# mp3guy/Kintinuous

Hardware: AMD Instinct MI355X
Metric: RGB-D frames/sec @640x480, 512^3 TSDF (higher is better)
Workload: dtype f32; 1 GPU; orbit512: 640x480 synthetic orbit sequence, ICP-only tracking, 512^3 TSDF, inputs resident in HBM, 1 stream per GPU (BASELINE.json configs[1]), log playback with 1 frame of read-ahead; volume=512, cols=640, rows=480, unique_frames=120, pose_gather_bytes=56384, side_gate=0, odometry_fallbacks=0

## Files before the change

kintinuous_amd/csrc/kt_track.hip:

```cpp
#include "kt_internal.hpp"

#include <string.h>
#include <stdlib.h>
#include <float.h>
#include <math.h>

#define KT_RED_THREADS 1024
#define KT_RED_BLOCKS 256
#define KT_VT_TOTAL 8192
#define KT_KBATCH 40
#define KT_P2_PAIRS 4
#define KT_RED_SLOTS 32

template <int CTRL>
__device__ __forceinline__ float kt_dpp(float v)
{
    return __int_as_float(__builtin_amdgcn_update_dpp(0, __float_as_int(v), CTRL, 0xf, 0xf, true));
}
__device__ __forceinline__ float kt_warp32_sum(float v)
{
    v += __int_as_float(__builtin_amdgcn_ds_swizzle(__float_as_int(v), 0x401F));
    v += kt_dpp<0x108>(v);
    v += kt_dpp<0x104>(v);
    v += kt_dpp<0x102>(v);
    v += kt_dpp<0x101>(v);
    return v;
}

__device__ __constant__ unsigned char KT_PA[28] = {0, 0, 0, 0, 0, 0, 0, 1, 1, 1, 1, 1, 1, 2, 2, 2, 2, 2, 3, 3, 3, 3, 4, 4, 4, 5, 5, 6};
__device__ __constant__ unsigned char KT_PB[28] = {0, 1, 2, 3, 4, 5, 6, 1, 2, 3, 4, 5, 6, 2, 3, 4, 5, 6, 3, 4, 5, 6, 4, 5, 6, 5, 6, 6};

struct kt_no_prefetch { __device__ __forceinline__ void operator()() const {} };
#define KT_RED_PAIRS 15
#define KT_GRANULE_SENTINEL 0xffffffffffffffffull
#define KT_LEVEL_SETS 2
#define KT_LEVEL_SET_STRIDE 4096
#define KT_LEVEL_SET_BASE 32768
#define KT_POSE_ABORT 15
__device__ __forceinline__ int kt_granule_index(int pair, int wg) { return pair * KT_RED_BLOCKS + (wg & 3) * (KT_RED_BLOCKS / 4) + (wg >> 2); }
__device__ __forceinline__ void kt_publish_pair(unsigned long long* __restrict__ granules, float wsum)
{
    unsigned int lo = __float_as_uint(wsum), hi = (unsigned int)__builtin_amdgcn_readlane((int)__float_as_uint(wsum), 32);
    lo = lo == 0xffffffffu ? 0xfffffffeu : lo;
    const int pair = threadIdx.x >> 6;
    if ((threadIdx.x & 63) == 0 && pair < KT_RED_PAIRS)
        __hip_atomic_store(&granules[kt_granule_index(pair, blockIdx.x)], ((unsigned long long)hi << 32) | (unsigned long long)lo, __ATOMIC_RELAXED,
                           __HIP_MEMORY_SCOPE_AGENT);
}
typedef float kt_rows_t[8][32][2];
static_assert(KT_KBATCH % (2 * KT_P2_PAIRS) == 0, "phase 2 reads whole groups of k-pairs: the staging array must hold them");

typedef float kt_f2 __attribute__((ext_vector_type(2)));
__device__ __forceinline__ float2 kt_lds_pair(const float (&p)[2])
{
    const kt_f2 w = *(const volatile __attribute__((address_space(3))) kt_f2*)p;
    return make_float2(w.x, w.y);
}
template <int NS>
__device__ __forceinline__ void kt_phase2(float (&acc)[NS], const kt_rows_t* const (&rows)[NS], int my_a, int my_b, int vt, int kcount, int kend)
{
    for (int j0 = 0; 2 * j0 < kcount; j0 += KT_P2_PAIRS) {
        float2 ra[KT_P2_PAIRS][NS], rb[KT_P2_PAIRS][NS];
#pragma unroll
        for (int u = 0; u < KT_P2_PAIRS; ++u)
#pragma unroll
            for (int s = 0; s < NS; ++s) {
                ra[u][s] = kt_lds_pair(rows[s][j0 + u][my_a][vt]);
                rb[u][s] = kt_lds_pair(rows[s][j0 + u][my_b][vt]);
            }
#pragma unroll
        for (int u = 0; u < KT_P2_PAIRS; ++u) {
            const int kl = 2 * (j0 + u);
#pragma unroll
            for (int s = 0; s < NS; ++s) acc[s] = kl < kend ? __builtin_fmaf(ra[u][s].x, rb[u][s].x, acc[s]) : acc[s];
#pragma unroll
            for (int s = 0; s < NS; ++s) acc[s] = kl + 1 < kend ? __builtin_fmaf(ra[u][s].y, rb[u][s].y, acc[s]) : acc[s];
        }
    }
}

template <typename RowFn>
__device__ __forceinline__ void kt_reduce29_publish(const RowFn& fn, int n, unsigned long long* __restrict__ granules, kt_rows_t* rows)
{
    KT_TS(0);
    const int tid = threadIdx.x;
    const int t0 = blockIdx.x * 32;
    const int comp = tid >> 5, vt = tid & 31;
    const int my_a = comp < 28 ? KT_PA[comp] : 7, my_b = comp < 28 ? KT_PB[comp] : 7;
    const int nk_vt = (n - (t0 + vt) + KT_VT_TOTAL - 1) / KT_VT_TOTAL;
    const int nk_blk = (n - t0 + KT_VT_TOTAL - 1) / KT_VT_TOTAL;
    float acc[1] = {0.f};
    const kt_rows_t* const rs[1] = {rows};
    for (int kb = 0; kb < nk_blk; kb += KT_KBATCH) {
        const int kcount = min(KT_KBATCH, nk_blk - kb);
        for (int p = tid; p < kcount * 32; p += 2 * KT_RED_THREADS) {
            const int p2 = p + KT_RED_THREADS;
            const int kl = p >> 5, v = p & 31, kl2 = p2 >> 5;
            const int i = t0 + v + (kb + kl) * KT_VT_TOTAL;
            const int i2 = t0 + v + (kb + kl2) * KT_VT_TOTAL;
            const bool has2 = p2 < kcount * 32;
            float row[7], row2[7];
            const bool found = fn(min(i, n - 1), row) && i < n;
            if (__builtin_amdgcn_ballot_w64(has2) != 0) {
                const bool found2 = fn(min(i2, n - 1), row2) && i2 < n && has2;
                if (has2) {
#pragma unroll
                    for (int q = 0; q < 7; ++q) rows[kl2 >> 1][q][v][kl2 & 1] = found2 ? row2[q] : 0.0f;
                    rows[kl2 >> 1][7][v][kl2 & 1] = found2 ? 1.0f : 0.0f;
                }
            }
#pragma unroll
            for (int q = 0; q < 7; ++q) rows[kl >> 1][q][v][kl & 1] = found ? row[q] : 0.0f;
            rows[kl >> 1][7][v][kl & 1] = found ? 1.0f : 0.0f;
        }
        __syncthreads();
        KT_TS_PHASE2(0);
        if (comp < 29) kt_phase2<1>(acc, rs, my_a, my_b, vt, kcount, min(kcount, nk_vt - kb));
        __syncthreads();
        KT_TS_PHASE2(1);
    }
    KT_TS(1);
    const float wsum = kt_warp32_sum(acc[0]);
    kt_publish_pair(granules, wsum);
    KT_TS(2);
}

template <typename RowFnA, typename RowFnB>
__device__ __forceinline__ void kt_reduce29_publish2(const RowFnA& fa, const RowFnB& fb, int n, unsigned long long* __restrict__ granules_a,
                                                     unsigned long long* __restrict__ granules_b, kt_rows_t* rows_a, kt_rows_t* rows_b)
{
    KT_TS(0);
    const int tid = threadIdx.x;
    const int t0 = blockIdx.x * 32;
    const int comp = tid >> 5, vt = tid & 31;
    const int my_a = comp < 28 ? KT_PA[comp] : 7, my_b = comp < 28 ? KT_PB[comp] : 7;
    const int nk_vt = (n - (t0 + vt) + KT_VT_TOTAL - 1) / KT_VT_TOTAL;
    const int nk_blk = (n - t0 + KT_VT_TOTAL - 1) / KT_VT_TOTAL;
    float acc[2] = {0.f, 0.f};
    const kt_rows_t* const rs[2] = {rows_a, rows_b};
    for (int kb = 0; kb < nk_blk; kb += KT_KBATCH) {
        const int kcount = min(KT_KBATCH, nk_blk - kb);
        for (int p = tid; p < kcount * 32; p += KT_RED_THREADS) {
            const int kl = p >> 5, v = p & 31;
            const int i = t0 + v + (kb + kl) * KT_VT_TOTAL;
            const int ii = min(i, n - 1);
            const auto term = fb.fetch_term(ii);
            f3 vcurr, ncurr, vcurr_g, vprev_g, nprev_g;
            bool inimg;
            int g;
            fa.fetch_curr(ii, vcurr, ncurr);
            typename RowFnB::taps tp;
            fb.fetch_taps(term, tp);
            fa.project(vcurr, vcurr_g, inimg, g);
            fa.fetch_prev(g, vprev_g, nprev_g);
            {
                float rb[7];
                const bool found_b = fb.finish(term, tp, rb) && i < n;
#pragma unroll
                for (int q = 0; q < 7; ++q) rows_b[kl >> 1][q][v][kl & 1] = found_b ? rb[q] : 0.0f;
                rows_b[kl >> 1][7][v][kl & 1] = found_b ? 1.0f : 0.0f;
            }
            float ra[7];
            const bool found_a = fa.finish(ncurr, vcurr_g, vprev_g, nprev_g, inimg, ra) && i < n;
#pragma unroll
            for (int q = 0; q < 7; ++q) rows_a[kl >> 1][q][v][kl & 1] = found_a ? ra[q] : 0.0f;
            rows_a[kl >> 1][7][v][kl & 1] = found_a ? 1.0f : 0.0f;
        }
        __syncthreads();
        KT_TS_PHASE2(0);
        if (comp < 29) kt_phase2<2>(acc, rs, my_a, my_b, vt, kcount, min(kcount, nk_vt - kb));
        __syncthreads();
        KT_TS_PHASE2(1);
    }
    KT_TS(1);
    const float wsum_a = kt_warp32_sum(acc[0]), wsum_b = kt_warp32_sum(acc[1]);
    kt_publish_pair(granules_a, wsum_a);
    kt_publish_pair(granules_b, wsum_b);
    KT_TS(2);
}

__device__ unsigned int kt_sweep_spin_limit = 1u << 22;
__device__ unsigned int kt_wait_limit_ticks = 5000000u;
__device__ __forceinline__ unsigned long long kt_ticks() { return __builtin_amdgcn_s_memrealtime(); }

template <int NS>
__device__ __forceinline__ void kt_reduce29_sweep_n(unsigned long long* const (&granules)[NS], float* const (&total)[NS], unsigned int patience = 40u)
{
    const int tid = threadIdx.x;
    KT_TS(3);
    __shared__ unsigned int timed_out;
    if (tid == 0) timed_out = 0;
    __syncthreads();
    {
        const int w = (tid >> 6) - 1, lane = tid & 63;
        if (w >= 0 && w < KT_RED_PAIRS) {
            unsigned long long g[NS][4];
            bool ok;
            unsigned int spins = 0;
            const unsigned int spin_limit = *(volatile const unsigned int*)&kt_sweep_spin_limit;
            const unsigned long long tick_limit = (unsigned long long)*(volatile const unsigned int*)&kt_wait_limit_ticks * patience;
            unsigned long long tick0 = 0;
            for (;;) {
#pragma unroll
                for (int s = 0; s < NS; ++s) {
                    const unsigned long long* pp = &granules[s][w * KT_RED_BLOCKS + lane];
#pragma unroll
                    for (int q = 0; q < 4; ++q) g[s][q] = __hip_atomic_load(pp + q * (KT_RED_BLOCKS / 4), __ATOMIC_RELAXED, __HIP_MEMORY_SCOPE_AGENT);
                }
                ok = true;
#pragma unroll
                for (int s = 0; s < NS; ++s)
#pragma unroll
                    for (int q = 0; q < 4; ++q) ok = ok && g[s][q] != KT_GRANULE_SENTINEL;
                if (__all(ok) || ++spins > spin_limit) break;
                if ((spins & 15u) == 0) {
                    const unsigned long long now = kt_ticks();
                    if (spins == 16u) tick0 = now;
                    else if (now - tick0 > tick_limit) break;
                }
                __builtin_amdgcn_s_sleep(1);
            }
            const bool all_ok = __all(ok);
            if (all_ok) {
#pragma unroll
                for (int s = 0; s < NS; ++s)
#pragma unroll
                    for (int q = 0; q < 4; ++q)
                        __hip_atomic_store(&granules[s][w * KT_RED_BLOCKS + lane + q * (KT_RED_BLOCKS / 4)], KT_GRANULE_SENTINEL, __ATOMIC_RELAXED, __HIP_MEMORY_SCOPE_AGENT);
            }
#pragma unroll
            for (int s = 0; s < NS; ++s)
#pragma unroll
                for (int r = 0; r < 2; ++r) {
                    const int c = 2 * w + r;
                    const float s0 = __uint_as_float((unsigned int)(g[s][0] >> (32 * r))) + 0.0f;
                    const float s1 = __uint_as_float((unsigned int)(g[s][1] >> (32 * r))) + 0.0f;
                    const float s2 = __uint_as_float((unsigned int)(g[s][2] >> (32 * r))) + 0.0f;
                    const float s3 = __uint_as_float((unsigned int)(g[s][3] >> (32 * r))) + 0.0f;
                    const float blk = (s0 + s2) + (s1 + s3);
                    const float tr = kt_warp32_sum(0.0f + blk);
                    const float lo = __int_as_float(__builtin_amdgcn_readlane(__float_as_int(tr), 0));
                    const float hi = __int_as_float(__builtin_amdgcn_readlane(__float_as_int(tr), 32));
                    if (lane == 0 && c < 29) total[s][c] = (lo + 0.0f) + (hi + 0.0f);
                }
            if (lane == 0 && !all_ok) atomicOr(&timed_out, 1u);
        }
    }
    __syncthreads();
    if (tid == 0) total[NS - 1][KT_RED_SLOTS - 1] = timed_out ? 1.0f : 0.0f;
    __syncthreads();
    KT_TS(4);
}

__device__ __forceinline__ void kt_reduce29_sweep(unsigned long long* __restrict__ granules, float (&total)[KT_RED_SLOTS], unsigned int patience = 40u)
{
    unsigned long long* const gs[1] = {granules};
    float* const ts[1] = {total};
    kt_reduce29_sweep_n<1>(gs, ts, patience);
}

#define KT_RED_GRID KT_RED_BLOCKS
__device__ __forceinline__ bool kt_red_publishes() { return true; }
__device__ __forceinline__ bool kt_red_sweeps() { return blockIdx.x == KT_RED_GRID - 1; }

template <typename RowFn, typename PreFn = kt_no_prefetch>
__device__ __forceinline__ bool kt_reduce29(const RowFn& fn, int n, unsigned long long* __restrict__ granules, float (&total)[KT_RED_SLOTS],
                                            const PreFn& pre = PreFn())
{
    __shared__ kt_rows_t rows[KT_KBATCH / 2];
    if (kt_red_publishes()) kt_reduce29_publish(fn, n, granules, rows);
    if (!kt_red_sweeps()) return false;
    pre();
    kt_reduce29_sweep(granules, total);
    return true;
}

int kt_refill_granules(kt_ctx* c)
{
    KT_HIP(hipMemsetAsync(c->red_partials, 0xff, sizeof(double) * 32 * c->red_max_blocks, c->stream));
    return KT_OK;
}

static unsigned int kt_next_epoch(kt_ctx* c)
{
    if (++c->red_epoch >= 0xffffffffu) {
        (void)kt_refill_granules(c);
        c->red_epoch = 1;
    }
    return c->red_epoch;
}
static unsigned long long* kt_residual_granules(kt_ctx* c) { return (unsigned long long*)c->red_partials + 64 * KT_RED_BLOCKS; }
static unsigned int* kt_residual_partials(kt_ctx* c) { return (unsigned int*)((unsigned long long*)c->red_partials + 64 * KT_RED_BLOCKS + 1024); }
static unsigned long long* kt_second_granules(kt_ctx* c) { return (unsigned long long*)c->red_partials + 32 * KT_RED_BLOCKS; }

struct kt_icp_args {
    const float* vmap_curr; const float* nmap_curr;
    const float* vmap_g_prev; const float* nmap_g_prev;
    kt_intr intr;
    int cols, rows;
    float dist_thres, angle_thres;
    float dist2_le, sine2_le;
    kt_mat33 Rcurr; float tcurr[3];
    kt_mat33 Rprev_inv; float tprev[3];
    kt_track_state* state;
    int first;
    unsigned long long* granules; unsigned int fault;
    float* out29;
    int mode;
    int keep29;
    int n_iter; unsigned int seq0; unsigned long long* pose_gran; unsigned long long* level_gran;
    int n_levels;
    struct level { const float* vmap_curr; const float* nmap_curr; const float* vmap_g_prev; const float* nmap_g_prev; kt_intr intr; int cols, rows, n_iter; } lv[KT_LEVELS];
};

struct kt_icp_row {
    struct view { const float* vmap_curr; const float* nmap_curr; const float* vmap_g_prev; const float* nmap_g_prev; kt_intr intr; int cols, rows; float dist2_le, sine2_le; } a;
    kt_mat33 Rcurr, Rprev_inv;
    f3 tcurr, tprev;
    __device__ __forceinline__ explicit kt_icp_row(const kt_icp_args& k)
        : a{k.vmap_curr, k.nmap_curr, k.vmap_g_prev, k.nmap_g_prev, k.intr, k.cols, k.rows, k.dist2_le, k.sine2_le} {}
    __device__ __forceinline__ void set_level(const kt_icp_args::level& v)
    {
        a.vmap_curr = v.vmap_curr; a.nmap_curr = v.nmap_curr; a.vmap_g_prev = v.vmap_g_prev; a.nmap_g_prev = v.nmap_g_prev;
        a.intr = v.intr; a.cols = v.cols; a.rows = v.rows;
    }
    int pf_i = -1;
    f3 pf_v = {0.f, 0.f, 0.f}, pf_n = {0.f, 0.f, 0.f};
    __device__ __forceinline__ void fetch_curr(int i, f3& vcurr, f3& ncurr) const
    {
        const int plane = a.cols * a.rows;
        vcurr = {a.vmap_curr[i], a.vmap_curr[i + plane], a.vmap_curr[i + 2 * plane]};
        ncurr = {a.nmap_curr[i], a.nmap_curr[i + plane], a.nmap_curr[i + 2 * plane]};
    }
    __device__ __forceinline__ void project(const f3& vcurr, f3& vcurr_g, bool& inimg, int& g) const
    {
        const int cols = a.cols, rows = a.rows;
        vcurr_g = kt_add(kt_mul(Rcurr, vcurr), tcurr);
        const f3 vcurr_cp = kt_mul(Rprev_inv, kt_sub(vcurr_g, tprev));
        const int ux = kt_f2i_rn(vcurr_cp.x * a.intr.fx / vcurr_cp.z + a.intr.cx);
        const int uy = kt_f2i_rn(vcurr_cp.y * a.intr.fy / vcurr_cp.z + a.intr.cy);
        inimg = !(ux < 0 || uy < 0 || ux >= cols || uy >= rows || vcurr_cp.z < 0);
        g = inimg ? (int)kt_mad24((unsigned int)uy, (unsigned int)cols, (unsigned int)ux) : 0;
    }
    __device__ __forceinline__ void fetch_prev(int g, f3& vprev_g, f3& nprev_g) const
    {
        const int plane = a.cols * a.rows;
        vprev_g = {a.vmap_g_prev[g], a.vmap_g_prev[g + plane], a.vmap_g_prev[g + 2 * plane]};
        nprev_g = {a.nmap_g_prev[g], a.nmap_g_prev[g + plane], a.nmap_g_prev[g + 2 * plane]};
    }
    __device__ __forceinline__ bool finish(const f3& ncurr, const f3& vcurr_g, const f3& vprev_g, const f3& nprev_g, bool inimg, float (&row)[7]) const
    {
        const f3 ncurr_g = kt_mul(Rcurr, ncurr);
        const f3 dv = kt_sub(vprev_g, vcurr_g);
        const float dist2 = kt_dot(dv, dv);
        const f3 cr = kt_cross(ncurr_g, nprev_g);
        const float sine2 = kt_dot(cr, cr);
        const bool found = inimg && (sine2 <= a.sine2_le && dist2 <= a.dist2_le && !kt_isnan(ncurr.x) && !kt_isnan(nprev_g.x));
        const f3 s_cp = kt_mul(Rprev_inv, kt_sub(vcurr_g, tprev));
        const f3 d_cp = kt_mul(Rprev_inv, kt_sub(vprev_g, tprev));
        const f3 n_cp = kt_mul(Rprev_inv, nprev_g);
        const f3 sxn = kt_cross(s_cp, n_cp);
        row[0] = found ? n_cp.x : 0.0f; row[1] = found ? n_cp.y : 0.0f; row[2] = found ? n_cp.z : 0.0f;
        row[3] = found ? sxn.x : 0.0f; row[4] = found ? sxn.y : 0.0f; row[5] = found ? sxn.z : 0.0f;
        row[6] = found ? kt_dot(n_cp, kt_sub(s_cp, d_cp)) : 0.0f;
        return found;
    }
    __device__ __forceinline__ bool operator()(int i, float (&row)[7]) const
    {
        f3 vcurr, ncurr, vcurr_g, vprev_g, nprev_g;
        bool inimg;
        int g;
        if (i == pf_i) { vcurr = pf_v; ncurr = pf_n; }
        else fetch_curr(i, vcurr, ncurr);
        project(vcurr, vcurr_g, inimg, g);
        fetch_prev(g, vprev_g, nprev_g);
        return finish(ncurr, vcurr_g, vprev_g, nprev_g, inimg, row);
    }
};

extern "C" float kt_debug_sq_threshold(float T, int strict)
{
    if (!(T >= 0.0f) || (strict && !(T > 0.0f))) return -1.0f;
    if (T == INFINITY) return strict ? FLT_MAX : INFINITY;
    const auto ok = [&](float x) { const float r = sqrtf(x); return strict ? r < T : r <= T; };
    float x = T * T;
    if (x == INFINITY) x = FLT_MAX;
    while (x > 0.0f && !ok(x)) x = nextafterf(x, -INFINITY);
    if (!ok(x)) return -1.0f;
    while (x < FLT_MAX && ok(nextafterf(x, INFINITY))) x = nextafterf(x, INFINITY);
    return x;
}
static void kt_icp_set_thresholds(kt_icp_args& a, float dist_thres, float angle_thres)
{
    a.dist_thres = dist_thres; a.angle_thres = angle_thres;
    a.dist2_le = kt_debug_sq_threshold(dist_thres, 0);
    a.sine2_le = kt_debug_sq_threshold(angle_thres, 1);
}

__global__ __launch_bounds__(KT_RED_THREADS) void kt_icp_kernel(const kt_icp_args a)
{
    if (a.fault && blockIdx.x == 0) return;
    kt_icp_row fn(a);
    if (a.state && !a.first) {
        for (int k = 0; k < 9; ++k) { fn.Rcurr.m[k] = a.state->Rcurr[k]; fn.Rprev_inv.m[k] = a.state->Rprev_inv[k]; }
        fn.tcurr = {a.state->tcurr[0], a.state->tcurr[1], a.state->tcurr[2]};
        fn.tprev = {a.state->tprev[0], a.state->tprev[1], a.state->tprev[2]};
    } else {
        fn.Rcurr = a.Rcurr; fn.Rprev_inv = a.Rprev_inv;
        fn.tcurr = {a.tcurr[0], a.tcurr[1], a.tcurr[2]};
        fn.tprev = {a.tprev[0], a.tprev[1], a.tprev[2]};
    }
    __shared__ float total[KT_RED_SLOTS];
    kt_pose_stage ps;
    const bool solve_here = a.mode == KT_MODE_ICP_SOLVE;
    auto pre = [&]() { if (solve_here && !a.first) ps.fetch(a.state); };
    if (!kt_reduce29(fn, a.cols * a.rows, a.granules, total, pre)) return;
    __shared__ double sys[KT_SYS_DOUBLES], pose_d[KT_POSE_STAGE_DOUBLES], tail_work[KT_TAIL_WORK_DOUBLES];
    __shared__ float pose_f[KT_POSE_STAGE_FLOATS];
    if (solve_here) {
        if (threadIdx.x < 42) sys[threadIdx.x] = (double)total[kt_sys_slot(threadIdx.x)];
        if (!a.first) ps.park(pose_d, pose_f);
        else if (threadIdx.x == 64) {
#pragma unroll
            for (int k = 0; k < 16; ++k) pose_d[k] = (k % 5 == 0) ? 1.0 : 0.0;
#pragma unroll
            for (int k = 0; k < 9; ++k) pose_f[k] = a.Rcurr.m[k];
#pragma unroll
            for (int k = 0; k < 3; ++k) pose_f[9 + k] = a.tprev[k];
        }
        __syncthreads();
    }
    if (a.mode == KT_MODE_HOST) {
        if (threadIdx.x < KT_RED_SLOTS && (threadIdx.x < 29 || threadIdx.x == KT_RED_SLOTS - 1)) a.out29[threadIdx.x] = total[threadIdx.x];
    } else if (a.mode == KT_MODE_ICP_SOLVE) {
        if (threadIdx.x == 64) {
            a.state->last_residual[0] = total[27];
            a.state->last_residual[1] = total[28];
            if (a.keep29)
                for (int k = 0; k < 29; ++k) a.state->icp29[k] = total[k];
            if (a.first) {
#pragma unroll
                for (int k = 0; k < 9; ++k) { a.state->Rprev[k] = a.Rcurr.m[k]; a.state->Rprev_inv[k] = a.Rprev_inv.m[k]; }
#pragma unroll
                for (int k = 0; k < 3; ++k) a.state->tprev[k] = a.tprev[k];
                a.state->handoff_timeout = total[KT_RED_SLOTS - 1] != 0.0f ? 1 : 0;
            } else if (total[KT_RED_SLOTS - 1] != 0.0f) {
                a.state->handoff_timeout = 1;
            }
        }
        if (threadIdx.x < 64) {
            kt_solve_and_update_wave(a.state, sys, pose_d, pose_f, tail_work);
#ifdef KT_ICP_TIMING
            if (threadIdx.x == 0) { const unsigned long long t5 = wall_clock64(); for (int q = 0; q < 7; ++q) a.state->icp29[q] = (float)(kt_ts[q + 0] - kt_ts[0]); a.state->icp29[7] = (float)(t5 - kt_ts[0]); }
#endif
        }
    } else if (threadIdx.x == 0) {
        for (int k = 0; k < 29; ++k) a.state->icp29[k] = total[k];
        if (total[KT_RED_SLOTS - 1] != 0.0f) a.state->handoff_timeout = 1;
    }
}


__device__ __forceinline__ void kt_level_wait_pose(const kt_icp_args& a, unsigned int want, float* s_pose)
{
    const int lane = (int)(threadIdx.x & 63u);
    const unsigned int spin_limit = min(*(volatile const unsigned int*)&kt_sweep_spin_limit, 1u << 20);
    const unsigned long long tick_limit = 2ull * *(volatile const unsigned int*)&kt_wait_limit_ticks;
    unsigned long long tick0 = 0;
    unsigned long long g = 0;
    unsigned int spins = 0;
    bool ok, gone;
    for (;;) {
        if (lane < 13) g = __hip_atomic_load(&a.pose_gran[lane == 12 ? KT_POSE_ABORT : lane], __ATOMIC_RELAXED, __HIP_MEMORY_SCOPE_AGENT);
        const int ahead = (int)((unsigned int)(g >> 32) - want);
        ok = lane >= 12 || ahead == 0;
        gone = lane == 12 && ahead >= 0 && ahead < a.n_iter;
        if (__all(ok) || __any(gone) || ++spins > spin_limit) break;
        if ((spins & 15u) == 0) {
            const unsigned long long now = kt_ticks();
            if (spins == 16u) tick0 = now;
// ... 844 lines not shown
```

Baseline: 4257 frames/s.

## Pack two outer-product components per thread in ICP reduction phase 2 with shared slot loads

Phase 2 of the 29-term ICP reduction now assigns each 64-lane wave two pairs of products, drawn from a constexpr table. Each thread loads three component slots and forms two FMAs from them, so LDS reads are shared across products instead of two loads per product. The loop is double-buffered with sched barriers and uses an inline-asm FMA. The per-thread kend bounds check is replaced by zero-padding the staging array in phase 1. Only 8 waves work in phase 2, which concentrates the work and adds table complexity and a padding pass.

New measurement: 4221 frames/s. About the same (-0.9%).

```diff
diff --git a/kintinuous_amd/csrc/kt_track.hip b/kintinuous_amd/csrc/kt_track.hip
--- a/kintinuous_amd/csrc/kt_track.hip
+++ b/kintinuous_amd/csrc/kt_track.hip
@@ -9,7 +9,7 @@
 #define KT_RED_BLOCKS 256
 #define KT_VT_TOTAL 8192
 #define KT_KBATCH 40
-#define KT_P2_PAIRS 4
+#define KT_P2_PAIRS 2
 #define KT_RED_SLOTS 32
 
 template <int CTRL>
@@ -27,8 +27,57 @@
     return v;
 }
 
-__device__ __constant__ unsigned char KT_PA[28] = {0, 0, 0, 0, 0, 0, 0, 1, 1, 1, 1, 1, 1, 2, 2, 2, 2, 2, 3, 3, 3, 3, 4, 4, 4, 5, 5, 6};
-__device__ __constant__ unsigned char KT_PB[28] = {0, 1, 2, 3, 4, 5, 6, 1, 2, 3, 4, 5, 6, 2, 3, 4, 5, 6, 3, 4, 5, 6, 4, 5, 6, 5, 6, 6};
+static constexpr unsigned char KT_PA[29] = {0, 0, 0, 0, 0, 0, 0, 1, 1, 1, 1, 1, 1, 2, 2, 2, 2, 2, 3, 3, 3, 3, 4, 4, 4, 5, 5, 6, 7};
+static constexpr unsigned char KT_PB[29] = {0, 1, 2, 3, 4, 5, 6, 1, 2, 3, 4, 5, 6, 2, 3, 4, 5, 6, 3, 4, 5, 6, 4, 5, 6, 5, 6, 6, 7};
+
+#define KT_P2_WAVES 8
+#define KT_P2_SLOTS 3
+struct kt_p2_wave {
+    unsigned char prod[2][2];
+    unsigned char comp[2][KT_P2_SLOTS];
+    signed char pair[2];
+};
+#define KT_P2_STAR {{0, 1}, {0, 2}}
+#define KT_P2_SQR {{0, 1}, {2, 2}}
+static constexpr kt_p2_wave KT_P2[KT_P2_WAVES] = {
+    {KT_P2_STAR, {{0, 0, 1}, {0, 2, 3}}, {0, 1}},
+    {KT_P2_STAR, {{0, 4, 5}, {1, 2, 3}}, {2, 4}},
+    {KT_P2_STAR, {{1, 4, 5}, {2, 3, 4}}, {5, 7}},
+    {KT_P2_STAR, {{2, 5, 6}, {3, 3, 4}}, {8, 9}},
+    {KT_P2_STAR, {{3, 5, 6}, {4, 4, 5}}, {10, 11}},
+    {KT_P2_SQR, {{0, 6, 1}, {1, 6, 2}}, {3, 6}},
+    {KT_P2_SQR, {{4, 6, 5}, {5, 6, 6}}, {12, 13}},
+    {KT_P2_SQR, {{7, 7, 7}, {7, 7, 7}}, {14, -1}},
+};
+constexpr int kt_p2_owner(int c)
+{
+    int owner = -1, n = 0;
+    for (int w = 0; w < KT_P2_WAVES; ++w)
+        for (int h = 0; h < 2; ++h)
+            for (int r = 0; r < 2; ++r) {
+                if (KT_P2[w].pair[h] < 0 || 2 * KT_P2[w].pair[h] + r != c) continue;
+                const unsigned char* pr = KT_P2[w].prod[r];
+                if (pr[0] >= KT_P2_SLOTS || pr[1] >= KT_P2_SLOTS) return -1;
+                if (KT_P2[w].comp[h][pr[0]] != KT_PA[c] || KT_P2[w].comp[h][pr[1]] != KT_PB[c]) return -1;
+                owner = w * 2 + h;
+                ++n;
+            }
+    return n == 1 ? owner : -1;
+}
+constexpr bool kt_p2_all_owned()
+{
+    for (int c = 0; c < 29; ++c)
+        if (kt_p2_owner(c) < 0) return false;
+    return true;
+}
+constexpr bool kt_p2_pairs_together()
+{
+    for (int p = 0; p < 14; ++p)
+        if (kt_p2_owner(2 * p) != kt_p2_owner(2 * p + 1)) return false;
+    return true;
+}
+static_assert(kt_p2_all_owned(), "every product 0..28 is formed exactly once, from slots that hold its two components");
+static_assert(kt_p2_pairs_together(), "products 2p and 2p + 1 share a thread: it stores their granule");
 
 struct kt_no_prefetch { __device__ __forceinline__ void operator()() const {} };
 #define KT_RED_PAIRS 15
@@ -38,44 +87,126 @@
 #define KT_LEVEL_SET_BASE 32768
 #define KT_POSE_ABORT 15
 __device__ __forceinline__ int kt_granule_index(int pair, int wg) { return pair * KT_RED_BLOCKS + (wg & 3) * (KT_RED_BLOCKS / 4) + (wg >> 2); }
-__device__ __forceinline__ void kt_publish_pair(unsigned long long* __restrict__ granules, float wsum)
-{
-    unsigned int lo = __float_as_uint(wsum), hi = (unsigned int)__builtin_amdgcn_readlane((int)__float_as_uint(wsum), 32);
+__device__ __forceinline__ void kt_publish_pair(unsigned long long* __restrict__ granules, int pair, float wsum_lo, float wsum_hi)
+{
+    unsigned int lo = __float_as_uint(wsum_lo);
+    const unsigned int hi = __float_as_uint(wsum_hi);
     lo = lo == 0xffffffffu ? 0xfffffffeu : lo;
-    const int pair = threadIdx.x >> 6;
-    if ((threadIdx.x & 63) == 0 && pair < KT_RED_PAIRS)
-        __hip_atomic_store(&granules[kt_granule_index(pair, blockIdx.x)], ((unsigned long long)hi << 32) | (unsigned long long)lo, __ATOMIC_RELAXED,
-                           __HIP_MEMORY_SCOPE_AGENT);
+    __hip_atomic_store(&granules[kt_granule_index(pair, blockIdx.x)], ((unsigned long long)hi << 32) | (unsigned long long)lo, __ATOMIC_RELAXED,
+                       __HIP_MEMORY_SCOPE_AGENT);
 }
 typedef float kt_rows_t[8][32][2];
 static_assert(KT_KBATCH % (2 * KT_P2_PAIRS) == 0, "phase 2 reads whole groups of k-pairs: the staging array must hold them");
 
 typedef float kt_f2 __attribute__((ext_vector_type(2)));
-__device__ __forceinline__ float2 kt_lds_pair(const float (&p)[2])
+__device__ __forceinline__ float2 kt_lds_pair(const float* p)
 {
     const kt_f2 w = *(const volatile __attribute__((address_space(3))) kt_f2*)p;
     return make_float2(w.x, w.y);
 }
+__device__ __forceinline__ float kt_fma(float a, float b, float acc)
+{
+    asm("v_fma_f32 %0, %1, %2, %0" : "+v"(acc) : "v"(a), "v"(b));
+    return acc;
+}
 template <int NS>
-__device__ __forceinline__ void kt_phase2(float (&acc)[NS], const kt_rows_t* const (&rows)[NS], int my_a, int my_b, int vt, int kcount, int kend)
-{
-    for (int j0 = 0; 2 * j0 < kcount; j0 += KT_P2_PAIRS) {
-        float2 ra[KT_P2_PAIRS][NS], rb[KT_P2_PAIRS][NS];
-#pragma unroll
-        for (int u = 0; u < KT_P2_PAIRS; ++u)
-#pragma unroll
-            for (int s = 0; s < NS; ++s) {
-                ra[u][s] = kt_lds_pair(rows[s][j0 + u][my_a][vt]);
-                rb[u][s] = kt_lds_pair(rows[s][j0 + u][my_b][vt]);
-            }
-#pragma unroll
-        for (int u = 0; u < KT_P2_PAIRS; ++u) {
-            const int kl = 2 * (j0 + u);
-#pragma unroll
-            for (int s = 0; s < NS; ++s) acc[s] = kl < kend ? __builtin_fmaf(ra[u][s].x, rb[u][s].x, acc[s]) : acc[s];
-#pragma unroll
-            for (int s = 0; s < NS; ++s) acc[s] = kl + 1 < kend ? __builtin_fmaf(ra[u][s].y, rb[u][s].y, acc[s]) : acc[s];
-        }
+__device__ __forceinline__ void kt_phase1_pad(kt_rows_t* const (&rows)[NS], int kcount)
+{
+    constexpr int G = KT_P2_PAIRS / NS;
+    static_assert(G >= 1 && KT_KBATCH % (2 * G) == 0, "phase 2 reads whole groups of k-pairs: the staging array must hold them");
+    const int kpad = (kcount + 2 * G - 1) / (2 * G) * (2 * G);
+    int z = KT_RED_THREADS - 1 - (int)threadIdx.x;
+    asm volatile("" : "+v"(z));
+    if (z < (kpad - kcount) * 32) {
+        const int kl = kcount + (z >> 5), v = z & 31;
+#pragma unroll
+        for (int s = 0; s < NS; ++s)
+#pragma unroll
+            for (int q = 0; q < 8; ++q) rows[s][kl >> 1][q][v][kl & 1] = 0.0f;
+    }
+}
+template <int W, int NS>
+__device__ __forceinline__ void kt_phase2_wave(float (&acc)[NS][2], const kt_rows_t* const (&rows)[NS], int half, int vt, int kcount)
+{
+    constexpr int NSLOT = KT_P2_SLOTS, G = KT_P2_PAIRS / NS;
+    const float* p[NS][NSLOT];
+#pragma unroll
+    for (int s = 0; s < NS; ++s)
+#pragma unroll
+        for (int q = 0; q < NSLOT; ++q)
+            p[s][q] = &rows[s][0][0][0][0] + (KT_P2[W].comp[0][q] * 32 + vt) * 2 + (-half & ((KT_P2[W].comp[1][q] - KT_P2[W].comp[0][q]) * 64));
+    constexpr int PAIR = 8 * 32 * 2;
+    const auto load = [&](float2 (&r)[G][NS][NSLOT], int j0) {
+#pragma unroll
+        for (int u = 0; u < G; ++u)
+#pragma unroll
+            for (int s = 0; s < NS; ++s)
+#pragma unroll
+                for (int q = 0; q < NSLOT; ++q) r[u][s][q] = kt_lds_pair(p[s][q] + (j0 + u) * PAIR);
+    };
+    const auto fold = [&](const float2 (&r)[G][NS][NSLOT]) {
+#pragma unroll
+        for (int u = 0; u < G; ++u) {
+#pragma unroll
+            for (int s = 0; s < NS; ++s)
+#pragma unroll
+                for (int i = 0; i < 2; ++i) acc[s][i] = kt_fma(r[u][s][KT_P2[W].prod[i][0]].x, r[u][s][KT_P2[W].prod[i][1]].x, acc[s][i]);
+#pragma unroll
+            for (int s = 0; s < NS; ++s)
+#pragma unroll
+                for (int i = 0; i < 2; ++i) acc[s][i] = kt_fma(r[u][s][KT_P2[W].prod[i][0]].y, r[u][s][KT_P2[W].prod[i][1]].y, acc[s][i]);
+        }
+    };
+    static_assert(2 * G <= KT_KBATCH / 2, "the two groups read up front lie inside the staging array");
+    float2 r0[G][NS][NSLOT], r1[G][NS][NSLOT];
+    load(r0, 0);
+    load(r1, G);
+#pragma nounroll
+    for (int j = 0;; j += 2 * G) {
+        __builtin_amdgcn_sched_barrier(0);
+        fold(r0);
+        if (2 * (j + G) >= kcount) break;
+        if (2 * (j + 2 * G) < kcount) load(r0, j + 2 * G);
+        __builtin_amdgcn_sched_barrier(0);
+        fold(r1);
+        if (2 * (j + 2 * G) >= kcount) break;
+        if (2 * (j + 3 * G) < kcount) load(r1, j + 3 * G);
+    }
+}
+template <int NS>
+__device__ __forceinline__ void kt_phase2(float (&acc)[NS][2], const kt_rows_t* const (&rows)[NS], int kcount)
+{
+    int lane = (int)threadIdx.x & 63;
+    asm volatile("" : "+v"(lane));
+    const int half = lane >> 5, vt = lane & 31;
+    switch (__builtin_amdgcn_readfirstlane((int)threadIdx.x >> 6)) {
+    case 0: kt_phase2_wave<0, NS>(acc, rows, half, vt, kcount); break;
+    case 1: kt_phase2_wave<1, NS>(acc, rows, half, vt, kcount); break;
+    case 2: kt_phase2_wave<2, NS>(acc, rows, half, vt, kcount); break;
+    case 3: kt_phase2_wave<3, NS>(acc, rows, half, vt, kcount); break;
+    case 4: kt_phase2_wave<4, NS>(acc, rows, half, vt, kcount); break;
+    case 5: kt_phase2_wave<5, NS>(acc, rows, half, vt, kcount); break;
+    case 6: kt_phase2_wave<6, NS>(acc, rows, half, vt, kcount); break;
+    case 7: kt_phase2_wave<7, NS>(acc, rows, half, vt, kcount); break;
+    default: break;
+    }
+}
+template <int NS>
+__device__ __forceinline__ void kt_phase2_publish(const float (&acc)[NS][2], unsigned long long* const (&granules)[NS])
+{
+    const int wave = __builtin_amdgcn_readfirstlane((int)threadIdx.x >> 6);
+    if (wave >= KT_P2_WAVES) return;
+    int lane = (int)threadIdx.x & 63;
+    asm volatile("" : "+v"(lane));
+    const int half = lane >> 5, vt = lane & 31;
+    int pair = 0;
+#pragma unroll
+    for (int w = 0; w < KT_P2_WAVES; ++w)
+        if (wave == w) pair = KT_P2[w].pair[0] + (-half & (KT_P2[w].pair[1] - KT_P2[w].pair[0]));
+#pragma unroll
+    for (int s = 0; s < NS; ++s) {
+        const float wsum0 = kt_warp32_sum(acc[s][0]), wsum1 = kt_warp32_sum(acc[s][1]);
+        if (vt == 0 && pair >= 0) kt_publish_pair(granules[s], pair, wsum0, 2 * pair + 1 < 29 ? wsum1 : 0.0f);
     }
 }
 
@@ -85,12 +216,11 @@
     KT_TS(0);
     const int tid = threadIdx.x;
     const int t0 = blockIdx.x * 32;
-    const int comp = tid >> 5, vt = tid & 31;
-    const int my_a = comp < 28 ? KT_PA[comp] : 7, my_b = comp < 28 ? KT_PB[comp] : 7;
-    const int nk_vt = (n - (t0 + vt) + KT_VT_TOTAL - 1) / KT_VT_TOTAL;
     const int nk_blk = (n - t0 + KT_VT_TOTAL - 1) / KT_VT_TOTAL;
-    float acc[1] = {0.f};
+    float acc[1][2] = {{0.f, 0.f}};
+    kt_rows_t* const rw[1] = {rows};
     const kt_rows_t* const rs[1] = {rows};
+    unsigned long long* const gs[1] = {granules};
     for (int kb = 0; kb < nk_blk; kb += KT_KBATCH) {
         const int kcount = min(KT_KBATCH, nk_blk - kb);
         for (int p = tid; p < kcount * 32; p += 2 * KT_RED_THREADS) {
@@ -113,15 +243,15 @@
             for (int q = 0; q < 7; ++q) rows[kl >> 1][q][v][kl & 1] = found ? row[q] : 0.0f;
             rows[kl >> 1][7][v][kl & 1] = found ? 1.0f : 0.0f;
         }
+        kt_phase1_pad<1>(rw, kcount);
         __syncthreads();
         KT_TS_PHASE2(0);
-        if (comp < 29) kt_phase2<1>(acc, rs, my_a, my_b, vt, kcount, min(kcount, nk_vt - kb));
+        kt_phase2<1>(acc, rs, kcount);
         __syncthreads();
         KT_TS_PHASE2(1);
     }
     KT_TS(1);
-    const float wsum = kt_warp32_sum(acc[0]);
-    kt_publish_pair(granules, wsum);
+    kt_phase2_publish<1>(acc, gs);
     KT_TS(2);
 }
 
@@ -132,12 +262,11 @@
     KT_TS(0);
     const int tid = threadIdx.x;
     const int t0 = blockIdx.x * 32;
-    const int comp = tid >> 5, vt = tid & 31;
-    const int my_a = comp < 28 ? KT_PA[comp] : 7, my_b = comp < 28 ? KT_PB[comp] : 7;
-    const int nk_vt = (n - (t0 + vt) + KT_VT_TOTAL - 1) / KT_VT_TOTAL;
     const int nk_blk = (n - t0 + KT_VT_TOTAL - 1) / KT_VT_TOTAL;
-    float acc[2] = {0.f, 0.f};
+    float acc[2][2] = {{0.f, 0.f}, {0.f, 0.f}};
+    kt_rows_t* const rw[2] = {rows_a, rows_b};
     const kt_rows_t* const rs[2] = {rows_a, rows_b};
+    unsigned long long* const gs[2] = {granules_a, granules_b};
     for (int kb = 0; kb < nk_blk; kb += KT_KBATCH) {
         const int kcount = min(KT_KBATCH, nk_blk - kb);
         for (int p = tid; p < kcount * 32; p += KT_RED_THREADS) {
@@ -166,16 +295,15 @@
             for (int q = 0; q < 7; ++q) rows_a[kl >> 1][q][v][kl & 1] = found_a ? ra[q] : 0.0f;
             rows_a[kl >> 1][7][v][kl & 1] = found_a ? 1.0f : 0.0f;
         }
+        kt_phase1_pad<2>(rw, kcount);
         __syncthreads();
         KT_TS_PHASE2(0);
-        if (comp < 29) kt_phase2<2>(acc, rs, my_a, my_b, vt, kcount, min(kcount, nk_vt - kb));
+        kt_phase2<2>(acc, rs, kcount);
         __syncthreads();
         KT_TS_PHASE2(1);
     }
     KT_TS(1);
-    const float wsum_a = kt_warp32_sum(acc[0]), wsum_b = kt_warp32_sum(acc[1]);
-    kt_publish_pair(granules_a, wsum_a);
-    kt_publish_pair(granules_b, wsum_b);
+    kt_phase2_publish<2>(acc, gs);
     KT_TS(2);
 }
 
```
